# 87003697/DynamiCrafter

Measured on AMD Instinct MI355X. Metric: frames/sec (and denoising-step ms), 16f@576x1024, DDIM 50, higher is better.
Workload: dtype bf16; 1 GPU; inference_1024_v1.0.yaml: 1 clip/GPU, 16 frames, latent 72x128, DDIM 50 uniform_trailing eta=1, CFG 7.5 batched (cond+uncond), guidance_rescale 0.7, v-param+ZTSNR+dynamic rescale, hipGraph-captured step; clips_per_gpu=1, parallelism=dp1 over 1 distinct clips (no data-path collective), conditioning=local (1 rank), outputs_finite=True

## Files before the change

### dynamicrafter_amd/_hip.py

```python
import ctypes as C
import os
import threading

_HERE = os.path.dirname(os.path.abspath(__file__))
LIB_PATH = os.environ.get("DC_HIP_LIB") or os.path.join(_HERE, "csrc", "libdcrafter_hip.so")

DC_GEMM_OUT_F32 = 1
DC_GEMM_GEGLU = 2
DC_GEMM_GELU = 4


class DcGemmParams(C.Structure):
    _fields_ = [
        ("A", C.c_void_p), ("W", C.c_void_p), ("C", C.c_void_p), ("bias", C.c_void_p),
        ("rowvec", C.c_void_p), ("residual", C.c_void_p),
        ("lda", C.c_int), ("ldc", C.c_int), ("ldr", C.c_int), ("rowvec_ld", C.c_int),
        ("rows_per_vec", C.c_int),
        ("M", C.c_int), ("N", C.c_int), ("K", C.c_int), ("n_pad", C.c_int),
        ("mode", C.c_int), ("Cin", C.c_int),
        ("IH", C.c_int), ("IW", C.c_int), ("OH", C.c_int), ("OW", C.c_int),
        ("stride", C.c_int), ("pad", C.c_int), ("ups", C.c_int),
        ("T", C.c_int), ("HW", C.c_int),
        ("flags", C.c_int), ("alpha", C.c_float),
        ("workspace", C.c_void_p), ("workspace_bytes", C.c_longlong),
# ... 47 lines not shown
    _fields_ = [
        ("c1", C.c_void_p), ("c2", C.c_void_p), ("w", C.c_void_p), ("step_size", C.c_void_p), ("bc2_sqrt", C.c_void_p),
        ("step_index", C.c_void_p), ("index", C.c_int), ("weight_type", C.c_int), ("x0_param", C.c_int),
        ("e_nchw", C.c_int), ("cfg_scale", C.c_float), ("guidance_rescale", C.c_float),
        ("beta2", C.c_float), ("eps", C.c_float), ("one_minus_beta1", C.c_float), ("one_minus_beta2", C.c_float),
        ("decay", C.c_float), ("grad_scale", C.c_float), ("noise_step_stride", C.c_int64), ("loss", C.c_void_p),
    ]


_P, _I, _F, _L = C.c_void_p, C.c_int, C.c_float, C.c_int64
SIGNATURES = {
    "dc_gemm_conv": (_I, [C.POINTER(DcGemmParams), _P]),
    "dc_gemm_fit": (_I, [C.POINTER(DcGemmParams), _P]),
    "dc_gemm_fit_shape": (_I, [_I, _I, _I]),
    "dc_gemm_workspace_bytes": (_L, []),
    "dc_gemm_last_variant": (C.c_char_p, []),
    "dc_gemm_set_plan": (_I, [_I]),
    "dc_groupnorm": (_I, [_P, _I, _P, _I, _P, _P, _I, _I, _I, _I, _F, _I, _P, _P]),
    "dc_groupnorm_workspace_bytes": (_L, [_I, _I, _I]),
    "dc_layernorm": (_I, [_P, _I, _P, _I, _P, _P, _I, _I, _F, _P]),
    "dc_ln_pool_tokens": (_I, [_P, _I, _P, _I, _P, _P, _I, _I, _I, _I, _I, _I, _F, _P]),
    "dc_flash_attn_d64": (_I, [_P, _P, _P, _P, _I, _I, _I, _I, _I, _I, _I, _I, _L, _L, _F, _I, _F, _P]),
    "dc_ff_geglu_fused320": (_I, [_P, _I, _P, _P, _F, _P, _P, _P, _P, _P, _I, _P, _I, _I, _P]),
    "dc_ff_geglu_proj_fused320": (_I, [_P, _I, _P, _P, _F, _P, _P, _P, _P, _P, _P, _P, _I, _P, _I, _I, _P]),
    "dc_ln_linear": (_I, [_P, _I, _I, _P, _P, _F, _P, _P, _P, _I, _I, _I, _P]),
    "dc_ln_qkv_temporal_attn320": (_I, [_P, _I, _P, _P, _F, _P, _P, _I, _I, _I, _I, _F, _P]),
    "dc_ln_qkv_temporal_attn640": (_I, [_P, _I, _P, _P, _F, _P, _P, _I, _I, _I, _I, _F, _P]),
    "dc_gn_silu_tconv3": (_I, [_P, _I, _I, _P, _P, _P, _I, _P, _P, _P, _I, _P, _I, _I, _I, _I, _I, _P]),
    "dc_groupnorm_stats": (_I, [_P, _I, _I, _I, _I, _I, _F, _P, _P, _P]),
    "dc_gn_linear": (_I, [_P, _I, _I, _P, _P, _P, _I, _I, _P, _P, _P, _I, _I, _I, _P]),
    "dc_flash_attn_set_mode": (_I, [_I, _F]),
    "dc_linear_residual": (_I, [_P, _I, _I, _P, _P, _P, _I, _P, _I, _I, _I, _P]),
    "dc_cross_attn_dual_d64": (_I, [_P, _P, _P, _P, _P, _P, _I, _I, _I, _I, _I, _I, _I, _I, _L, _L, _F, _F, _P]),
    "dc_temporal_attn_d64": (_I, [_P, _I, _P, _I, _I, _I, _I, _I, _F, _P]),
    "dc_gemv_small": (_I, [_P, _I, _P, _P, _P, _I, _I, _I, _I, _I, _I, _I, _P]),
    "dc_timestep_embedding": (_I, [_P, _P, _I, _P, _I, _I, _F, _P]),
    "dc_pack_latent": (_I, [_P, _P, _P, _I, _I, _I, _I, _I, _I, _I, _P]),
    "dc_pack_latent_windows": (_I, [_P, _P, _P, _P, _P] + [_I] * 13 + [_P]),
    "dc_window_merge": (_I, [_P, _I, _P, _I, _P, _P, _P] + [_I] * 12 + [_P]),
    "dc_pack_latent_tiles": (_I, [_P, _P, _P, _P, _P] + [_I] * 16 + [_P]),
    "dc_tile_merge": (_I, [_P, _I, _P, _I, _P, _P, _P] + [_I] * 15 + [_P]),
    "dc_nchw_to_rows": (_I, [_P, _P, _I, _I, _I, _I, _F, _P]),
    "dc_rows_to_nchw": (_I, [_P, _I, _I, _P, _I, _I, _I, _F, _P]),
    "dc_im2col3x3_c8": (_I, [_P, _I, _P, _I, _I, _I, _I, _P]),
    "dc_copy2d": (_I, [_P, _I, _P, _I, _I, _I, _P]),
    "dc_build_context": (_I, [_P, _P, _I, _I, _I, _I, _I, _P]),
    "dc_softmax_rows": (_I, [_P, _I, _P, _I, _I, _I, _P]),
    "dc_transpose": (_I, [_P, _I, _P, _I, _I, _I, _P]),
    "dc_add_rows": (_I, [_P, _I, _P, _I, _P, _I, _I, _I, _P]),
    "dc_vae_sample": (_I, [_P, _I, _P, _P, _I, _I, _I, _F, _P]),
    "dc_ddim_step": (_I, [C.POINTER(DcDdimParams), _P, _P, _P, _I, _P, _P, _P, _P, _I, _I, _I, _P, _P]),
    "dc_ddim_invert_step": (_I, [C.POINTER(DcInvertParams), _P, _P, _P, _I, _P, _P, _P, _I, _I, _I, _P, _P]),
    "dc_dpmpp_step": (_I, [C.POINTER(DcDpmParams), _P, _P, _P, _I, _P, _P, _P, _P, _I, _I, _I, _P, _P]),
    "dc_sds_noise": (_I, [C.POINTER(DcSdsParams), _P, _P, _P, _I, _L, _P]),
    "dc_sds_step": (_I, [C.POINTER(DcSdsParams), _P, _P, _I, _P, _P, _P, _P, _I, _I, _I, _P, _P]),
    "dc_attn_small": (_I, [_P, _P, _P, _P, _I, _I, _I, _I, _I, _I, _I, _I, _I, _F, _I, _P]),
    "dc_attn_small_lds_bytes": (_L, [_I, _I]),
    "dc_clip_preprocess": (_I, [_P, _P, _P, _P, _I, _I, _I, _I, _I, _I, _I, C.POINTER(_F), C.POINTER(_F), _P]),
    "dc_patchify": (_I, [_P, _P, _I, _I, _I, _I, _I, _I, _P]),
    "dc_embed_tokens": (_I, [_P, _P, _P, _P, _I, _I, _I, _I, _P]),
    "dc_frames_to_u8": (_I, [_P, _P, _I, _I, _I, _I, _I, _P]),
    "dc_jpeg_dct_quant": (_I, [_P, _P, _P, _I, _I, _I, _P]),
    "dc_jpeg_entropy": (_I, [_P, _P, _P, _I, _I, _I, _I, _L, _P]),
    "dc_jpeg_pack": (_I, [_P, _P, _P, _P, _P, _I, _I, _L, _L, _P]),
    "dc_jpeg_decode_entropy": (_I, [_P, _L, _P, _P, _P, _P, _P] + [_I] * 8 + [_P]),
    "dc_jpeg_decode_idct": (_I, [_P, _P, _P] + [_I] * 6 + [_P]),
# ... 79 lines not shown
```

### dynamicrafter_amd/csrc/attn_parts.h

```cpp
#pragma once
#include "dc_common.h"
#include "lds_stage.h"

namespace {

constexpr int ATTN_VLD = 192;

__device__ __forceinline__ int attn_key_of(int j0, int r, int fh) { return j0 + (r & 3) + 8 * (r >> 2) + 4 * fh; }
__device__ __forceinline__ bf16x8_t attn_q_scaled(const u32x4_t& raw, float c) {
    u32x4_t sc;
#pragma unroll
    for (int e = 0; e < 4; ++e) sc[e] = pack_bf2(__uint_as_float(raw[e] << 16) * c, __uint_as_float(raw[e] & 0xffff0000u) * c);
    return __builtin_bit_cast(bf16x8_t, sc);
}
__device__ __forceinline__ bf16x8_t attn_pack_p(const f32x16_t& s, int ks) {
    u32x4_t pw;
#pragma unroll
    for (int e = 0; e < 4; ++e) pw[e] = pack_bf2(s[8 * ks + 2 * e], s[8 * ks + 2 * e + 1]);
    return __builtin_bit_cast(bf16x8_t, pw);
}
__device__ __forceinline__ int attn_vt_lane_off(int lane) {
    const int li = lane & 15;
    return (li >> 2) * ATTN_VLD + (((lane >> 4) & 1) * 16 + (li & 3) * 4) * 2;
}
__device__ __forceinline__ bf16x8_t attn_vt_join(const bf16x4_t lo, const bf16x4_t hi) {
    bf16x8_t vf;
    vf[0] = lo[0]; vf[1] = lo[1]; vf[2] = lo[2]; vf[3] = lo[3];
    vf[4] = hi[0]; vf[5] = hi[1]; vf[6] = hi[2]; vf[7] = hi[3];
    return vf;
}
__device__ __forceinline__ bf16x8_t attn_vt_frag(const lds_char_t* vp) {
    const bf16x4_t lo = __builtin_amdgcn_ds_read_tr16_b64_v4i16((lds_bf16x4_t*)(vp));
    const bf16x4_t hi = __builtin_amdgcn_ds_read_tr16_b64_v4i16((lds_bf16x4_t*)(vp + 8 * ATTN_VLD));
    return attn_vt_join(lo, hi);
}
__device__ __forceinline__ void attn_stage_row(char* sk, char* sv, int r, int chunk, const u32x4_t& kreg, const u32x4_t& vreg) {
    *reinterpret_cast<u32x4_t*>(sk + lds_off128(r, chunk)) = kreg;
    *reinterpret_cast<u32x4_t*>(sv + r * ATTN_VLD + chunk * 16) = vreg;
}
__device__ __forceinline__ void attn_store_row(bf16_t* orow, bool live, int fh, const f32x16_t (&f)[2]) {
#pragma unroll
    for (int db = 0; db < 2; ++db)
#pragma unroll
        for (int qd = 0; qd < 4; qd += 2) {
            const unsigned a0 = pack_bf2(f[db][4 * qd + 0], f[db][4 * qd + 1]);
            const unsigned a1 = pack_bf2(f[db][4 * qd + 2], f[db][4 * qd + 3]);
            const unsigned b0 = pack_bf2(f[db][4 * qd + 4], f[db][4 * qd + 5]);
            const unsigned b1 = pack_bf2(f[db][4 * qd + 6], f[db][4 * qd + 7]);
            const auto r0 = __builtin_amdgcn_permlane32_swap(a0, b0, false, false);
            const auto r1 = __builtin_amdgcn_permlane32_swap(a1, b1, false, false);
            const u32x4_t pk = {r0[0], r1[0], r0[1], r1[1]};
            if (live) *reinterpret_cast<u32x4_t*>(orow + db * 32 + 8 * (qd + fh)) = pk;
        }
}

}
```

### dynamicrafter_amd/csrc/ff_fused.hip

```cpp
#include "attn_parts.h"
#include "dc_common.h"
#include "dcrafter_hip.h"
#include "lds_stage.h"
#include <stdint.h>
#include <type_traits>

namespace {

constexpr int FD = 320;
constexpr int FM = 4 * FD;
constexpr int FCH = 32;
constexpr int FNCH = FM / FCH;
constexpr int FBM = 128;
constexpr int W1_STAGE = 64 * FD * 2;
constexpr int W2_STAGE = FD * FCH * 2;
constexpr int W2_RING = 3;
constexpr int FF_LDS = 2 * W1_STAGE + W2_RING * W2_STAGE + 4 * 2048 + 2 * FM * 4;
static_assert(FF_LDS <= 160 * 1024, "LDS");

#ifdef DC_FF_STAMPS
__device__ unsigned long long g_ff_stamps[8];
#define FF_STAMP(i) do { asm volatile("s_waitcnt lgkmcnt(0)" ::: "memory"); const unsigned long long t__ = __builtin_readcyclecounter(); \
                         st_acc[i] += t__ - st_last; st_last = t__; } while (0)
#else
// ... 936 lines not shown
                                                     : __builtin_amdgcn_update_dpp(0, __float_as_int(yv), 0x101, 0xf, 0xf, false));
                }
            }
        }
        {
            const int n0 = c * LCH;
            const int rrow = lane >> 2, rc = lane & 3;
            if constexpr (RES) {
                if constexpr (KH != 1) {
#pragma unroll
                    for (int t = 0; t < 2; ++t) rres[t] = *reinterpret_cast<const u32x4_t*>(p.R + grow(t * 16 + rrow) * p.ldr + n0 + rc * 8);
                }
#pragma unroll
                for (int t = 0; t < 2; ++t) *xs_patch_row(ebuf, t * 16 + rrow, rc) = rres[t];
            }
#pragma unroll
            for (int q = 0; q < 4; ++q) {
                float4 bv = bias_lds ? *reinterpret_cast<const float4*>(bls + n0 + 8 * q + 4 * fh)
                                     : *reinterpret_cast<const float4*>(p.bias + n0 + 8 * q + 4 * fh);
                uint2* const slot2 = xs_patch_acc(ebuf, fr, fh, q);
                if constexpr (RES) xs_add_bf16x4(bv, *slot2);
                *slot2 = xs_pack_acc(out, q, bv);
            }
#pragma unroll
            for (int t = 0; t < 2; ++t) {
                const int r = t * 16 + rrow;
                const u32x4_t d = *xs_patch_row(ebuf, r, rc);
                *reinterpret_cast<u32x4_t*>(p.O + grow(r) * p.ldo + n0 + rc * 8) = d;
            }
        }
    }
}

}

#ifdef DC_FF_STAMPS
extern "C" int dc_ff_debug_stamps(unsigned long long* out, int reset) {
    hipError_t e = hipMemcpyFromSymbol(out, HIP_SYMBOL(g_ff_stamps), sizeof(unsigned long long) * 8);
    if (e == hipSuccess && reset) {
        unsigned long long z[8] = {0};
        e = hipMemcpyToSymbol(HIP_SYMBOL(g_ff_stamps), z, sizeof(z));
    }
    return (int)e;
}
#endif

template <bool LN, bool PROJ>
static int launch_ff_fused(const FfParams& p, hipStream_t stream) {
    static DcLdsOnce lds_once;
    if (const int e = lds_once.ensure(reinterpret_cast<const void*>(&ff_geglu_fused320_kernel<LN, PROJ>), FF_LDS)) return e;
    const int tiles = (p.M + FBM - 1) / FBM;
    hipLaunchKernelGGL((ff_geglu_fused320_kernel<LN, PROJ>), dim3(tiles < 256 ? tiles : 256), dim3(256), FF_LDS, stream, p);
    DC_CHECK_LAUNCH();
    return 0;
}

static int ff_fused_common(const uint16_t* x, int ldx, const float* ln_gamma, const float* ln_beta, float ln_eps,
                           const uint16_t* w1, const float* b1, const uint16_t* w2p, const float* b2, const uint16_t* residual,
                           int ldr, uint16_t* out, int ldo, const uint16_t* wp, const float* bp, const uint16_t* residual2,
                           int ldr2, uint16_t* out2, int ldo2, int M, hipStream_t stream) {
    FfParams p;
    p.X = x; p.ldx = ldx; p.W1 = w1; p.b1 = b1; p.W2p = w2p; p.b2 = b2; p.R = residual; p.ldr = ldr; p.O = out; p.ldo = ldo;
    p.M = M; p.ln_g = ln_gamma; p.ln_b = ln_beta; p.ln_eps = ln_eps;
    p.Wp = wp; p.bp = bp; p.R2 = residual2; p.ldr2 = ldr2; p.O2 = out2; p.ldo2 = ldo2;
    if (wp) return ln_gamma ? launch_ff_fused<true, true>(p, stream) : launch_ff_fused<false, true>(p, stream);
    return ln_gamma ? launch_ff_fused<true, false>(p, stream) : launch_ff_fused<false, false>(p, stream);
// ... 50 lines not shown
    }
    if (norm == 1) return launch_norm_linear_t<1, 2>(p, grid, stream);
    if (norm == 2) return launch_norm_linear_t<2, 2>(p, grid, stream);
    return launch_norm_linear_t<0, 2>(p, grid, stream);
}

static int ll_params(LlParams& p, const uint16_t* x, int ldx, int K, const uint16_t* w, const float* bias, uint16_t* out, int ldo,
                     int M, int N) {
    if ((K != FD && K != 2 * FD) || M < 1 || N < LCH || N % LCH || ldx % 8 || ldo % 8) return DC_ERR_SHAPE;
    if (((uintptr_t)x | (uintptr_t)out | (uintptr_t)w) % 16) return DC_ERR_SHAPE;
    p.X = x; p.ldx = ldx; p.W = w; p.bias = bias; p.O = out; p.ldo = ldo; p.M = M; p.N = N;
    p.ln_g = nullptr; p.ln_b = nullptr; p.ln_eps = 0.f; p.gn_stats = nullptr; p.gn_groups = 1; p.gn_rpi = FBM;
    p.R = nullptr; p.ldr = 0;
    return 0;
}

extern "C" int dc_ln_linear(const uint16_t* x, int ldx, int K, const float* ln_gamma, const float* ln_beta, float ln_eps,
                            const uint16_t* w, const float* bias, uint16_t* out, int ldo, int M, int N, void* stream_) {
    if (!x || !w || !out || ((ln_gamma == nullptr) != (ln_beta == nullptr))) return DC_ERR_ARG;
    LlParams p;
    if (const int e = ll_params(p, x, ldx, K, w, bias, out, ldo, M, N)) return e;
    p.ln_g = ln_gamma; p.ln_b = ln_beta; p.ln_eps = ln_eps;
    return launch_norm_linear(ln_gamma ? 1 : 0, K, p, (hipStream_t)stream_);
}

extern "C" int dc_linear_residual(const uint16_t* x, int ldx, int K, const uint16_t* w, const float* bias,
                                  const uint16_t* residual, int ldr, uint16_t* out, int ldo, int M, int N, void* stream_) {
    if (!x || !w || !out || !residual) return DC_ERR_ARG;
    LlParams p;
    if (const int e = ll_params(p, x, ldx, K, w, bias, out, ldo, M, N)) return e;
    if (ldr % 8 || (uintptr_t)residual % 16) return DC_ERR_SHAPE;
    p.R = residual; p.ldr = ldr;
    return launch_norm_linear(0, K, p, (hipStream_t)stream_);
}

extern "C" int dc_gn_linear(const uint16_t* x, int ldx, int K, const float* gamma, const float* beta, const float* stats,
                            int groups, int rows_per_inst, const uint16_t* w, const float* bias, uint16_t* out, int ldo,
                            int M, int N, void* stream_) {
    if (!x || !w || !out || !gamma || !beta || !stats) return DC_ERR_ARG;
    LlParams p;
    if (const int e = ll_params(p, x, ldx, K, w, bias, out, ldo, M, N)) return e;
    if (groups < 1 || K % groups || rows_per_inst < FBM || rows_per_inst % FBM || M % rows_per_inst) return DC_ERR_SHAPE;
    p.ln_g = gamma; p.ln_b = beta;
    p.gn_stats = reinterpret_cast<const float2*>(stats); p.gn_groups = groups; p.gn_rpi = rows_per_inst;
    return launch_norm_linear(2, K, p, (hipStream_t)stream_);
}

template <int KH>
static int launch_ln_qkv_tattn(const uint16_t* x, int ldx, const float* ln_gamma, const float* ln_beta, float ln_eps,
                               const uint16_t* wqkv, uint16_t* out, int ldo, int B, int T, int HW, float scale, void* stream_) {
    if (!x || !ln_gamma || !ln_beta || !wqkv || !out) return DC_ERR_ARG;
    if (B < 1 || T != 16 || HW < 8 || HW % 8 || ldx % 8 || ldo % 8) return DC_ERR_SHAPE;
    if (((uintptr_t)x | (uintptr_t)out | (uintptr_t)wqkv) % 16) return DC_ERR_SHAPE;
    static DcLdsOnce lds_once;
    if (const int e = lds_once.ensure(reinterpret_cast<const void*>(&ln_qkv_tattn_kernel<KH>), ta_lds(KH))) return e;
    TaParams p;
    p.X = x; p.ldx = ldx; p.W = wqkv; p.O = out; p.ldo = ldo; p.ln_g = ln_gamma; p.ln_b = ln_beta; p.ln_eps = ln_eps;
    p.HW = HW; p.c = scale * 1.4426950408889634f;
    static const int hsplit_env = [] { const char* e = getenv("DC_TA_HSPLIT"); return e ? atoi(e) : 0; }();
    const int hsplit = (KH == 2 && hsplit_env == 2) ? 2 : 1;
    hipLaunchKernelGGL(ln_qkv_tattn_kernel<KH>, dim3((unsigned)(B * (HW / 8)), hsplit), dim3(256), ta_lds(KH), (hipStream_t)stream_, p);
    DC_CHECK_LAUNCH();
    return 0;
}

extern "C" int dc_ln_qkv_temporal_attn320(const uint16_t* x, int ldx, const float* ln_gamma, const float* ln_beta, float ln_eps,
// ... 40 lines not shown
```

### dynamicrafter_amd/lvdm/modules/networks/openaimodel3d.py

```python
import math

import torch
import torch.nn as nn

from .... import ops
from ....ops import PackedWeight
from ....param_tree import attach_params

import os

_BF16 = torch.bfloat16
_FF_FUSED = os.environ.get("DC_FF_FUSED", "1") != "0"
_LN_FUSED = os.environ.get("DC_LN_FUSED", "1") != "0"
_LR_FUSED = os.environ.get("DC_LR_FUSED", "1") != "0"
_TA_FUSED = os.environ.get("DC_TA_FUSED", "1") != "0"
_TA_FUSED_C = tuple(int(k) for k in os.environ.get("DC_TA_FUSED_C", "320,640").split(","))
_FFP_FUSED = os.environ.get("DC_FFP_FUSED", "1") != "0"
_TC_FUSED = os.environ.get("DC_TC_FUSED", "1") != "0"
_GEMM_FIT = os.environ.get("DC_GEMM_FIT", "1") != "0"
_FIT_ROUTES = {
    (1280, 1280): "61 / 86 [gemm_persist_kernel<128>]; with residual 79 / 95; same bits",
    (3840, 1280): "168 / 207 [gemm_persist_kernel<320>]; same bits",
}
_FIT_MEASURED_NOT_ROUTED = {
    (1280, 5120): "213 / 255 [gemm_pipe320x16_kernel+splitk]",
    (640, 2560): "251 / 316 [gemm_pipe320x16_kernel+splitk]",
    (1280, 1920): "78 / 123 [gemm_pipe320x16_kernel+splitk]",
    (1280, 2560): "100 / 143 [gemm_pipe320x16_kernel+splitk]",
}


def _linear(a, pw, out, residual=None):
    if _GEMM_FIT and (pw.N, pw.K) in _FIT_ROUTES and ops.gemm_fits(out.shape[0], pw):
        return ops.gemm_fit(a, pw, out, residual=residual)
    return ops.gemm(a, pw, out, residual=residual)
_FUSED_MIN_ROWS = int(os.environ.get("DC_FUSED_MIN_ROWS", "4096"))
_LN_FUSED_K = tuple(int(k) for k in os.environ.get("DC_LN_FUSED_K", "320,640").split(","))
C_IN_PAD = 64


def _block_layout(cfg):
    mc, mults, nrb = cfg["model_channels"], list(cfg["channel_mult"]), cfg["num_res_blocks"]
    attn_res = set(cfg["attention_resolutions"])
    hc = cfg["num_head_channels"]
    tconv = bool(cfg["temporal_conv"])

    def transformers(ch):
        out = [("spatial", {"ch": ch, "heads": ch // hc})]
        if cfg["temporal_attention"]:
            out.append(("temporal", {"ch": ch, "inner": ch, "heads": ch // hc, "linear": bool(cfg["use_linear"])}))
        return out
# ... 511 lines not shown
    def _ff_proj(self, W, h, x, out):
        B_ = W["blk"]
        if "proj_p" in W and _FF_FUSED and _FFP_FUSED and h.shape[0] >= _FUSED_MIN_ROWS:
            return ops.ff_geglu_proj_fused320(h, B_["ff1"], B_["ff2p"], B_["ff2"].bias, W["proj_p"], W["proj_out"].bias, x, out,
                                              ln=B_["norm3"], ln_eps=1e-5)
        h = self._ff(B_, h)
        return self._lin_res(h, W["proj_out"], x, out)

    def _spatial_pre(self, W, x, g, heads):
        A = self._arena
        M, dev, Cc = x.shape[0], x.device, x.shape[1]
        h = self._gn_linear(x, W["norm"], W["proj_in"], A.get("tr_h", M, Cc, device=dev), n_inst=g["F"], rpi=g["HW"])
        B_ = W["blk"]
        return self._attn_self_spatial(B_["attn1"], B_["norm1"], h, g, heads)

    def _context_kv(self, B_, ctx, tag):
        return ops.gemm(ctx, B_["kv_ctx"], self._arena.get(tag, ctx.shape[0], B_["kv_ctx"].N, device=ctx.device))

    def precompute_context_kv(self, ctx_rows):
        Wt = self.packed(ctx_rows.device)
        down_path, middle, up_path = self._layout
        out = {"__gen__": Wt["gen"]}
        for name, blks, Ws in (("in", down_path, Wt["in"]), ("mid", [middle], [Wt["mid"]]), ("out", up_path, Wt["out"])):
            for i, (blk, Wb) in enumerate(zip(blks, Ws)):
                for j, ((kind, a), W) in enumerate(zip(blk, Wb)):
                    if kind == "spatial":
                        out[W["blk"]["key"]] = self._context_kv(W["blk"], ctx_rows, f"kvctx.{name}{i}.{j}")
        return out

    def _spatial_post(self, W, x, h, g, heads, out_tag, out=None):
        A = self._arena
        M, dev, Cc = x.shape[0], x.device, x.shape[1]
        B_ = W["blk"]
        q = self._ln_linear(h, B_["norm2"], B_["q2"], A.get("q2", M, Cc, device=dev))
        kv = None if g.get("ctx_kv") is None else g["ctx_kv"].get(B_["key"])
        if kv is None:
            kv = self._context_kv(B_, g["ctx"], "kvctx")
        att = A.get("att", M, Cc, device=dev)
        Lc, nt = g["Lc"], g["n_text"]
        if self.image_cross_attention and Lc > nt:
            ops.cross_attn_dual(q, kv[:, :Cc], kv[:, Cc:2 * Cc], kv[nt:, 2 * Cc:3 * Cc], kv[nt:, 3 * Cc:], att, batch=g["F"],
                                heads=heads, Lq=g["HW"], Lk=nt, Lk2=Lc - nt, scale=0.125, scale2=B_["ip_scale"], kv_bstride=Lc)
        else:
            ops.flash_attn(q, kv[:, :Cc], kv[:, Cc:2 * Cc], att, batch=g["F"], heads=heads, Lq=g["HW"], Lk=nt, scale=0.125,
                           kv_bstride=Lc)
        h = self._lin_res(att, B_["out2"], h, h)
        return self._ff_proj(W, h, x, out if out is not None else A.get(out_tag, M, Cc, device=dev))

    def _spatial(self, W, x, g, heads, out_tag, out=None):
        return self._spatial_post(W, x, self._spatial_pre(W, x, g, heads), g, heads, out_tag, out=out)

    def _temporal(self, W, x, g, heads, out_tag, out=None):
        A = self._arena
        M, dev, Cc = x.shape[0], x.device, x.shape[1]
        inner = W["proj_in"].N
        h = self._gn_linear(x, W["norm"], W["proj_in"], A.get("tr_h", M, inner, device=dev), n_inst=g["B"],
                            rpi=g["T"] * g["HW"])
        B_ = W["blk"]
        h = self._attn_self_temporal(B_["attn1"], B_["norm1"], h, g, heads)
        h = self._attn_self_temporal(B_["attn2"], B_["norm2"], h, g, heads)
        return self._ff_proj(W, h, x, out if out is not None else A.get(out_tag, M, Cc, device=dev))

    def _run_block(self, blk, Wb, h, g, tag, final=None):
        A = self._arena
        for j, ((kind, a), W) in enumerate(zip(blk, Wb)):
            out_tag = f"{tag}.{j}"
            dev = h.device
            last = final is not None and j == len(blk) - 1
            if kind == "conv_in":
                conv = dict(IH=g["H"], IW=g["W"], OH=g["H"], OW=g["W"], stride=1, pad=1, ups=0)
                dst = final(h.shape[0], a["cout"]) if last else A.get(out_tag, h.shape[0], a["cout"], device=dev)
                if "lin8" in W:
# ... 186 lines not shown
```

### dynamicrafter_amd/ops.py

```python
import ctypes as C
import os
import math

import torch

from . import _hip
from ._hip import DcDdimParams, DcGemmParams, check

_BF16 = torch.bfloat16


def stream_ptr():
    return C.c_void_p(torch.cuda.current_stream().cuda_stream)


class Tracer:

    def __init__(self):
        self.records = []

    def __enter__(self):
        global _TRACE
        _TRACE = self
        return self
# ... 440 lines not shown
    _launch("ff_geglu_proj_fused320", 2.0 * M * (2560 + 1280 + 320) * 320, 2.0 * M * 320 * 3 + 2.0 * (2560 * 320 + 320 * 1280 + 320 * 320),
            _hip.lib().dc_ff_geglu_proj_fused320, _ptr(x), x.stride(0), _ptr(None if ln is None else ln[0]),
            _ptr(None if ln is None else ln[1]), ln_eps, _ptr(pw1.w), _ptr(pw1.bias), _ptr(w2p), _ptr(b2), _ptr(wp), _ptr(bp),
            _ptr(residual2), residual2.stride(0), _ptr(out), out.stride(0), M, stream_ptr())
    return out


def ln_linear(x, pw, out, ln=None, ln_eps=1e-5):
    _rows(x, "x"); _rows(out, "out")
    M, K = x.shape[0], pw.K
    if K not in (320, 640) or pw.N % 32:
        raise ValueError("ln_linear: K must be 320 or 640 and N a multiple of 32")
    _need_rows(x, M, K, "x"); _need_rows(out, M, pw.N, "out")
    if ln is not None:
        _need(ln[0], K, "ln gamma"); _need(ln[1], K, "ln beta")
    _launch("ln_linear", 2.0 * M * pw.N * K, 2.0 * M * (K + pw.N) + 2.0 * pw.N * K, _hip.lib().dc_ln_linear,
            _ptr(x), x.stride(0), K, _ptr(None if ln is None else ln[0]), _ptr(None if ln is None else ln[1]), ln_eps,
            _ptr(pw.w), _ptr(pw.bias), _ptr(out), out.stride(0), M, pw.N, stream_ptr())
    return out


def linear_residual(x, pw, residual, out):
    _rows(x, "x"); _rows(out, "out"); _rows(residual, "residual")
    M, K = x.shape[0], pw.K
    if K not in (320, 640) or pw.N % 32:
        raise ValueError("linear_residual: K must be 320 or 640 and N a multiple of 32")
    _need_rows(x, M, K, "x"); _need_rows(out, M, pw.N, "out"); _need_rows(residual, M, pw.N, "residual")
    _launch("linear_residual", 2.0 * M * pw.N * K, 2.0 * M * (K + 2 * pw.N) + 2.0 * pw.N * K, _hip.lib().dc_linear_residual,
            _ptr(x), x.stride(0), K, _ptr(pw.w), _ptr(pw.bias), _ptr(residual), residual.stride(0), _ptr(out), out.stride(0),
            M, pw.N, stream_ptr())
    return out


def ln_qkv_temporal_attn(x, ln, pw_qkv, out, *, B, T, HW, scale, ln_eps=1e-5):
    _rows(x, "x"); _rows(out, "out")
    M = B * T * HW
    Cc = pw_qkv.K
    if Cc not in (320, 640) or pw_qkv.N != 3 * Cc or pw_qkv.bias is not None or T != 16 or HW % 8:
        raise ValueError("ln_qkv_temporal_attn: dim 320 / 640 (qkv weight [3 C, C], no bias), T = 16, HW % 8 == 0")
    if x.data_ptr() == out.data_ptr():
        raise ValueError("ln_qkv_temporal_attn: out must not alias x")
    _need_rows(x, M, Cc, "x"); _need_rows(out, M, Cc, "out"); _need(ln[0], Cc, "ln gamma"); _need(ln[1], Cc, "ln beta")
    fn = _hip.lib().dc_ln_qkv_temporal_attn320 if Cc == 320 else _hip.lib().dc_ln_qkv_temporal_attn640
    _launch(f"ln_qkv_temporal_attn{Cc}", 2.0 * M * 3 * Cc * Cc + 4.0 * M * T * Cc, 4.0 * M * Cc + 2.0 * 3 * Cc * Cc,
            fn, _ptr(x), x.stride(0), _ptr(ln[0]), _ptr(ln[1]), ln_eps, _ptr(pw_qkv.w),
            _ptr(out), out.stride(0), B, T, HW, scale, stream_ptr())
    return out


def gn_silu_tconv3(x, gamma, beta, stats, pw, out, *, B, T, HW, groups=32, residual=None):
    _rows(x, "x"); _rows(out, "out")
    M = B * T * HW
    C = pw.w.shape[1] // 3
    if C not in (320, 640) or pw.w.shape[1] != 3 * C or pw.N % 32 or pw.bias is None or T != 16 or HW % 8:
        raise ValueError("gn_silu_tconv3: 320 / 640 input channels (weight [N, 3 C] with bias), N % 32 == 0, T = 16, HW % 8 == 0")
    if x.data_ptr() == out.data_ptr():
        raise ValueError("gn_silu_tconv3: out must not alias x")
    _need_rows(x, M, C, "x"); _need_rows(out, M, pw.N, "out")
    _need(gamma, C, "gamma"); _need(beta, C, "beta"); _need(stats, B * groups * 2, "stats")
    if residual is not None:
        _rows(residual, "residual"); _need_rows(residual, M, pw.N, "residual")
    _launch("gn_silu_tconv3", 2.0 * M * pw.N * 3 * C, 2.0 * M * (C + pw.N * (2 if residual is not None else 1)) + 2.0 * pw.N * 3 * C,
            _hip.lib().dc_gn_silu_tconv3, _ptr(x), x.stride(0), C, _ptr(gamma), _ptr(beta), _ptr(stats), groups, _ptr(pw.w),
            _ptr(pw.bias), _ptr(residual), 0 if residual is None else residual.stride(0), _ptr(out), out.stride(0), B, T, HW,
            pw.N, stream_ptr())
    return out
# ... 1099 lines not shown
```

### include/dcrafter_hip.h

```cpp
#ifndef DCRAFTER_HIP_H
#define DCRAFTER_HIP_H
#include <stdint.h>

#ifdef __cplusplus
extern "C" {
#endif

#define DC_ERR_SHAPE (-1)
#define DC_ERR_ARG   (-2)

#define DC_GEMM_OUT_F32 1
#define DC_GEMM_GEGLU   2
#define DC_GEMM_GELU    4

typedef struct DcGemmParams {
    const uint16_t* A;
    const uint16_t* W;
    void* C;
    const float* bias;
    const float* rowvec;
    const uint16_t* residual;
    int lda, ldc, ldr, rowvec_ld;
    int rows_per_vec;
    int M, N, K, n_pad;
// ... 172 lines not shown
    float grad_scale;
    int64_t noise_step_stride;
    float* loss;
} DcSdsParams;

int dc_sds_noise(const DcSdsParams* p, const float* latent, const float* noise, float* x_t, int B, int64_t n_per_clip,
                 void* stream);

int dc_sds_step(const DcSdsParams* p, const float* e_cond, const float* e_uncond, int ld_e, const float* x_t,
                float* latent, float* m, float* v, int B, int C, int THW, float* workspace, void* stream);

int dc_cross_attn_dual_d64(const uint16_t* q, const uint16_t* k, const uint16_t* v, const uint16_t* k2, const uint16_t* v2,
                           uint16_t* o, int ldq, int ldkv, int ldo, int batch, int heads, int Lq, int Lk, int Lk2,
                           int64_t q_bstride, int64_t kv_bstride, float scale, float scale2, void* stream);

int dc_ff_geglu_fused320(const uint16_t* x, int ldx, const float* ln_gamma, const float* ln_beta, float ln_eps,
                         const uint16_t* w1, const float* b1, const uint16_t* w2p, const float* b2, const uint16_t* residual,
                         int ldr, uint16_t* out, int ldo, int M, void* stream);

int dc_ff_geglu_proj_fused320(const uint16_t* x, int ldx, const float* ln_gamma, const float* ln_beta, float ln_eps,
                              const uint16_t* w1, const float* b1, const uint16_t* w2p, const float* b2, const uint16_t* wp,
                              const float* bp, const uint16_t* residual2, int ldr2, uint16_t* out, int ldo, int M, void* stream);

int dc_ln_linear(const uint16_t* x, int ldx, int K, const float* ln_gamma, const float* ln_beta, float ln_eps, const uint16_t* w,
                 const float* bias, uint16_t* out, int ldo, int M, int N, void* stream);
int dc_groupnorm_stats(const uint16_t* x, int ldx, int C, int groups, int n_inst, int rows_per_inst, float eps,
                       float* workspace, float* stats_out, void* stream);
int dc_gn_linear(const uint16_t* x, int ldx, int K, const float* gamma, const float* beta, const float* stats, int groups,
                 int rows_per_inst, const uint16_t* w, const float* bias, uint16_t* out, int ldo, int M, int N, void* stream);

int dc_linear_residual(const uint16_t* x, int ldx, int K, const uint16_t* w, const float* bias, const uint16_t* residual, int ldr,
                       uint16_t* out, int ldo, int M, int N, void* stream);

int dc_ln_qkv_temporal_attn320(const uint16_t* x, int ldx, const float* ln_gamma, const float* ln_beta, float ln_eps,
                               const uint16_t* wqkv, uint16_t* out, int ldo, int B, int T, int HW, float scale, void* stream);
int dc_ln_qkv_temporal_attn640(const uint16_t* x, int ldx, const float* ln_gamma, const float* ln_beta, float ln_eps,
                               const uint16_t* wqkv, uint16_t* out, int ldo, int B, int T, int HW, float scale, void* stream);

int dc_gn_silu_tconv3(const uint16_t* x, int ldx, int C, const float* gamma, const float* beta, const float* stats, int groups,
                      const uint16_t* w, const float* bias, const uint16_t* residual, int ldr, uint16_t* out, int ldo, int B, int T,
                      int HW, int N, void* stream);


int dc_attn_small(const uint16_t* q, const uint16_t* k, const uint16_t* v, uint16_t* o, int ldq, int ldk, int ldv, int ldo,
                  int B, int heads, int Lq, int Lk, int d, float scale, int causal, void* stream);
int64_t dc_attn_small_lds_bytes(int Lk, int d);

int dc_clip_preprocess(const float* img, float* tmp0, float* tmp1, float* out, int N, int C, int H, int W, int OH, int OW,
                       int antialias, const float* mean3, const float* std3, void* stream);

int dc_patchify(const float* img, uint16_t* rows, int N, int C, int H, int W, int p, int kpad, void* stream);

int dc_embed_tokens(const int64_t* tokens, const uint16_t* table, const uint16_t* pos, uint16_t* out, int B, int L, int D,
                    int vocab, void* stream);

int dc_frames_to_u8(const float* video, uint8_t* out, int N, int C, int T, int H, int W, void* stream);


#define DC_JPEG_MCU_MAX_BYTES 2496

int dc_jpeg_dct_quant(const uint8_t* frames, const uint8_t* qtab, int16_t* coef, int T, int H, int W, void* stream);

int dc_jpeg_entropy(const int16_t* coef, uint8_t* scratch, int32_t* seg_len, int T, int my, int mx, int ri, int64_t stride,
                    void* stream);

int dc_jpeg_pack(const uint8_t* scratch, const int32_t* seg_len, int32_t* seg_off, uint8_t* out, int32_t* frame_len, int T,
// ... 129 lines not shown
```

Baseline: 2.590 frames/s.

## Fuse LN, Q projection, dual cross-attention and output projection for C=320 blocks

Adds one kernel that handles the C=320 spatial-transformer cross-attention block. Per 128-row tile it applies LayerNorm, the to_q GEMM, text plus image dual cross-attention with K/V staged in LDS, the to_out GEMM, the bias and the residual add. This removes the q and attention-output round trips to HBM and two kernel launches per block. The cost is a large register- and LDS-heavy kernel that loops over heads serially and may lose occupancy compared with the separate kernels. It is gated by shape conditions (Lk in 65..96, image tokens at most 32, HW divisible by 128).

Result: no change. 2.608 frames/s (median of 6 runs) (+0.7%).

```diff
diff --git a/dynamicrafter_amd/_hip.py b/dynamicrafter_amd/_hip.py
--- a/dynamicrafter_amd/_hip.py
+++ b/dynamicrafter_amd/_hip.py
@@ -103,6 +103,8 @@
     "dc_flash_attn_set_mode": (_I, [_I, _F]),
     "dc_linear_residual": (_I, [_P, _I, _I, _P, _P, _P, _I, _P, _I, _I, _I, _P]),
     "dc_cross_attn_dual_d64": (_I, [_P, _P, _P, _P, _P, _P, _I, _I, _I, _I, _I, _I, _I, _I, _L, _L, _F, _F, _P]),
+    "dc_xattn_block_fused320": (_I, [_P, _I, _P, _P, _F, _P, _P, _P, _P, _P, _P, _I, _L, _I, _I, _F, _F, _P, _P, _P, _I,
+                                     _I, _I, _I, _I, _P]),
     "dc_temporal_attn_d64": (_I, [_P, _I, _P, _I, _I, _I, _I, _I, _F, _P]),
     "dc_gemv_small": (_I, [_P, _I, _P, _P, _P, _I, _I, _I, _I, _I, _I, _I, _P]),
     "dc_timestep_embedding": (_I, [_P, _P, _I, _P, _I, _I, _F, _P]),
diff --git a/dynamicrafter_amd/csrc/attn_parts.h b/dynamicrafter_amd/csrc/attn_parts.h
--- a/dynamicrafter_amd/csrc/attn_parts.h
+++ b/dynamicrafter_amd/csrc/attn_parts.h
@@ -38,6 +38,11 @@
     *reinterpret_cast<u32x4_t*>(sk + lds_off128(r, chunk)) = kreg;
     *reinterpret_cast<u32x4_t*>(sv + r * ATTN_VLD + chunk * 16) = vreg;
 }
+__device__ __forceinline__ u32x4_t attn_swap_piece(unsigned a0, unsigned a1, unsigned b0, unsigned b1) {
+    const auto r0 = __builtin_amdgcn_permlane32_swap(a0, b0, false, false);
+    const auto r1 = __builtin_amdgcn_permlane32_swap(a1, b1, false, false);
+    return u32x4_t{r0[0], r1[0], r0[1], r1[1]};
+}
 __device__ __forceinline__ void attn_store_row(bf16_t* orow, bool live, int fh, const f32x16_t (&f)[2]) {
 #pragma unroll
     for (int db = 0; db < 2; ++db)
@@ -47,9 +52,7 @@
             const unsigned a1 = pack_bf2(f[db][4 * qd + 2], f[db][4 * qd + 3]);
             const unsigned b0 = pack_bf2(f[db][4 * qd + 4], f[db][4 * qd + 5]);
             const unsigned b1 = pack_bf2(f[db][4 * qd + 6], f[db][4 * qd + 7]);
-            const auto r0 = __builtin_amdgcn_permlane32_swap(a0, b0, false, false);
-            const auto r1 = __builtin_amdgcn_permlane32_swap(a1, b1, false, false);
-            const u32x4_t pk = {r0[0], r1[0], r0[1], r1[1]};
+            const u32x4_t pk = attn_swap_piece(a0, a1, b0, b1);
             if (live) *reinterpret_cast<u32x4_t*>(orow + db * 32 + 8 * (qd + fh)) = pk;
         }
 }
diff --git a/dynamicrafter_amd/csrc/ff_fused.hip b/dynamicrafter_amd/csrc/ff_fused.hip
--- a/dynamicrafter_amd/csrc/ff_fused.hip
+++ b/dynamicrafter_amd/csrc/ff_fused.hip
@@ -992,6 +992,230 @@
     }
 }
 
+
+constexpr int XB_K1 = 0, XB_V1 = 96 * 128, XB_K2 = XB_V1 + 96 * ATTN_VLD, XB_V2 = XB_K2 + 32 * 128, XB_KV = XB_V2 + 32 * ATTN_VLD;
+static_assert(XB_KV <= 2 * LW_STAGE, "a head's K / V sets alias the weight ring");
+constexpr int XB_LDS = 2 * LW_STAGE + 4 * 2048 + 2 * FD * 4 + 2 * FD * 4;
+
+struct XbParams {
+    const bf16_t* X; int ldx;
+    const float* ln_g; const float* ln_b; float ln_eps;
+    const bf16_t* Wq; const float* bq;
+    const bf16_t* K1; const bf16_t* V1; const bf16_t* K2; const bf16_t* V2; int ldkv; int64_t kv_bstride; int Lk, Lk2;
+    float c;
+    float acc_scale;
+    const bf16_t* Wo; const float* bo;
+    bf16_t* O; int ldo;
+    int HW;
+};
+
+__global__ __launch_bounds__(256, 2)
+void xattn_block320_kernel(const XbParams p) {
+    extern __shared__ __attribute__((aligned(16))) char smem[];
+    const int tid = threadIdx.x;
+    const int lane = tid & 63;
+    const int wave = __builtin_amdgcn_readfirstlane(tid >> 6);
+    const int fr = lane & 31, fh = lane >> 5;
+    const unsigned lds_base = (unsigned)(unsigned long)((lds_char_t*)smem);
+    char* const ebuf = smem + 2 * LW_STAGE + wave * 2048;
+    float* const lns = reinterpret_cast<float*>(smem + 2 * LW_STAGE + 4 * 2048);
+    float* const bqs = lns + 2 * FD;
+    float* const bos = bqs + FD;
+    const int tile = xcd_remap(blockIdx.x, gridDim.x);
+    const int frame = (tile * FBM) / p.HW;
+    const XsRowsLinear rows{tile * FBM + wave * 32, (int)gridDim.x * FBM};
+
+    unsigned vo[5];
+    xs_piece_offsets<FD * 2, 128>(vo, wave, lane);
+    auto w_base = [&](const bf16_t* W, int c) { return (uint64_t)(uintptr_t)W + (uint64_t)c * (LCH * FD * 2); };
+    xs_issue_stage(lds_base, 0, wave, vo, w_base(p.Wq, 0));
+
+    u32x4_t qa[FD / 16];
+    constexpr int PD = 6;
+    {
+        bf16x8_t xf[FD / 16];
+        xs_load_rows(xf, p.X + rows(fr) * p.ldx + fh * 8);
+        xs_stage_ln_affine(lns, FD, p.ln_g, p.ln_b, tid);
+        if (p.bq) xs_stage_bias(bqs, p.bq, FD, tid);
+        if (p.bo) xs_stage_bias(bos, p.bo, FD, tid);
+        asm volatile("s_waitcnt vmcnt(0) lgkmcnt(0)" ::: "memory");
+        __builtin_amdgcn_s_barrier();
+        asm volatile("" ::: "memory");
+        ln_rows_inplace<FD>(xf, lns, lns + FD, p.ln_eps, fh);
+#pragma unroll
+        for (int c = 0; c < FD / LCH; ++c) {
+            if (c > 0) {
+                wait_vmcnt<0>();
+                __builtin_amdgcn_s_barrier();
+                asm volatile("" ::: "memory");
+            }
+            f32x16_t acc;
+#pragma unroll
+            for (int r = 0; r < 16; ++r) acc[r] = 0.f;
+            const bool more = c + 1 < FD / LCH;
+            const uint64_t nb = w_base(p.Wq, c + 1);
+            xs_stage_mma<PD>(smem + (c & 1) * LW_STAGE, xf, 0, acc, fr, fh, [&](int i) __attribute__((always_inline)) {
+                if (more) lds_dma16_sbase(xs_stage_dst(lds_base, ((c & 1) ^ 1) * LW_STAGE, wave, i), vo[i], nb);
+            });
+#pragma unroll
+            for (int qd = 0; qd < 4; qd += 2) {
+                float4 bv0 = {0.f, 0.f, 0.f, 0.f}, bv1 = {0.f, 0.f, 0.f, 0.f};
+                if (p.bq) {
+                    bv0 = *reinterpret_cast<const float4*>(bqs + c * LCH + 8 * qd + 4 * fh);
+                    bv1 = *reinterpret_cast<const float4*>(bqs + c * LCH + 8 * (qd + 1) + 4 * fh);
+                }
+                const uint2 a = xs_pack_acc(acc, qd, bv0), b = xs_pack_acc(acc, qd + 1, bv1);
+                qa[2 * c + (qd >> 1)] = attn_swap_piece(a.x, a.y, b.x, b.y);
+            }
+        }
+    }
+
+    const int tr_off = attn_vt_lane_off(lane);
+    auto scores = [&](const char* sk, int nkeys, auto NB_, f32x16_t (&s)[3], const bf16x8_t (&qf)[4]) __attribute__((always_inline)) -> float {
+        constexpr int NB = decltype(NB_)::value;
+#pragma unroll
+        for (int jb = 0; jb < NB; ++jb) {
+#pragma unroll
+            for (int r = 0; r < 16; ++r) s[jb][r] = 0.f;
+#pragma unroll
+            for (int kk = 0; kk < 4; ++kk) {
+                const bf16x8_t kf = *reinterpret_cast<const bf16x8_t*>(sk + lds_off128(jb * 32 + fr, kk * 2 + fh));
+                s[jb] = __builtin_amdgcn_mfma_f32_32x32x16_bf16(kf, qf[kk], s[jb], 0, 0, 0);
+            }
+        }
+#pragma unroll
+        for (int r = 0; r < 16; ++r)
+            if (attn_key_of((NB - 1) * 32, r, fh) >= nkeys) s[NB - 1][r] = -1e30f;
+        float mx = s[0][0];
+#pragma unroll
+        for (int jb = 0; jb < NB; ++jb)
+#pragma unroll
+            for (int r = 0; r < 16; ++r) mx = fmaxf(mx, s[jb][r]);
+        mx = fmaxf(mx, __shfl_xor(mx, 32, 64));
+        float sum = 0.f;
+#pragma unroll
+        for (int jb = 0; jb < NB; ++jb)
+#pragma unroll
+            for (int r = 0; r < 16; ++r) {
+                const float pv = __builtin_amdgcn_exp2f(s[jb][r] - mx);
+                s[jb][r] = pv;
+                sum += pv;
+            }
+        return sum + __shfl_xor(sum, 32, 64);
+    };
+    auto pv_mma = [&](const char* sv, auto NB_, const f32x16_t (&s)[3], f32x16_t (&oacc)[2]) __attribute__((always_inline)) {
+        constexpr int NB = decltype(NB_)::value;
+#pragma unroll
+        for (int jb = 0; jb < NB; ++jb)
+#pragma unroll
+            for (int ks = 0; ks < 2; ++ks) {
+                const int jbase = jb * 32 + 16 * ks + 4 * fh;
+                const bf16x8_t pf = attn_pack_p(s[jb], ks);
+#pragma unroll
+                for (int db = 0; db < 2; ++db) {
+                    const bf16x8_t vf = attn_vt_frag((const lds_char_t*)(sv + jbase * ATTN_VLD + db * 64 + tr_off));
+                    oacc[db] = __builtin_amdgcn_mfma_f32_32x32x16_bf16(vf, pf, oacc[db], 0, 0, 0);
+                }
+            }
+    };
+    {
+        const int chunk = tid & 7, srow = tid >> 3;
+        const size_t kvrow0 = (size_t)frame * p.kv_bstride;
+#pragma unroll
+        for (int head = 0; head < FD / 64; ++head) {
+            u32x4_t kr[4], vr[4];
+#pragma unroll
+            for (int i = 0; i < 3; ++i) {
+                int j = srow + 32 * i;
+                j = j < p.Lk ? j : p.Lk - 1;
+                kr[i] = *reinterpret_cast<const u32x4_t*>(p.K1 + (kvrow0 + j) * p.ldkv + head * 64 + chunk * 8);
+                vr[i] = *reinterpret_cast<const u32x4_t*>(p.V1 + (kvrow0 + j) * p.ldkv + head * 64 + chunk * 8);
+            }
+            {
+                const int j = srow < p.Lk2 ? srow : p.Lk2 - 1;
+                kr[3] = *reinterpret_cast<const u32x4_t*>(p.K2 + (kvrow0 + j) * p.ldkv + head * 64 + chunk * 8);
+                vr[3] = *reinterpret_cast<const u32x4_t*>(p.V2 + (kvrow0 + j) * p.ldkv + head * 64 + chunk * 8);
+            }
+            __builtin_amdgcn_s_barrier();
+            asm volatile("" ::: "memory");
+#pragma unroll
+            for (int i = 0; i < 3; ++i) attn_stage_row(smem + XB_K1, smem + XB_V1, srow + 32 * i, chunk, kr[i], vr[i]);
+            attn_stage_row(smem + XB_K2, smem + XB_V2, srow, chunk, kr[3], vr[3]);
+            __syncthreads();
+
+            bf16x8_t qf[4];
+#pragma unroll
+            for (int kk = 0; kk < 4; ++kk) qf[kk] = attn_q_scaled(qa[4 * head + kk], p.c);
+            f32x16_t s[3], o1[2], o2[2];
+#pragma unroll
+            for (int d = 0; d < 2; ++d)
+#pragma unroll
+                for (int r = 0; r < 16; ++r) { o1[d][r] = 0.f; o2[d][r] = 0.f; }
+            const float l1 = scores(smem + XB_K1, p.Lk, ic<3>{}, s, qf);
+            pv_mma(smem + XB_V1, ic<3>{}, s, o1);
+            const float l2 = scores(smem + XB_K2, p.Lk2, ic<1>{}, s, qf);
+            pv_mma(smem + XB_V2, ic<1>{}, s, o2);
+            const float w1 = 1.0f / l1, w2 = p.acc_scale / l2;
+#pragma unroll
+            for (int db = 0; db < 2; ++db)
+#pragma unroll
+                for (int qd = 0; qd < 4; qd += 2) {
+                    float f[8];
+#pragma unroll
+                    for (int e = 0; e < 8; ++e) f[e] = __builtin_fmaf(o1[db][4 * qd + e], w1, o2[db][4 * qd + e] * w2);
+                    const unsigned a0 = pack_bf2(f[0], f[1]), a1 = pack_bf2(f[2], f[3]);
+                    const unsigned b0 = pack_bf2(f[4], f[5]), b1 = pack_bf2(f[6], f[7]);
+                    qa[4 * head + 2 * db + (qd >> 1)] = attn_swap_piece(a0, a1, b0, b1);
+                }
+        }
+    }
+
+    {
+        bf16x8_t xf[FD / 16];
+#pragma unroll
+        for (int kk = 0; kk < FD / 16; ++kk) xf[kk] = __builtin_bit_cast(bf16x8_t, qa[kk]);
+        __builtin_amdgcn_s_barrier();
+        asm volatile("" ::: "memory");
+        xs_issue_stage(lds_base, 0, wave, vo, w_base(p.Wo, 0));
+        int slot = 0;
+        for (int c = 0; c < FD / LCH; ++c) {
+            if (c == 0) wait_vmcnt<0>();
+            else wait_vmcnt<2>();
+            __builtin_amdgcn_s_barrier();
+            asm volatile("" ::: "memory");
+            f32x16_t acc;
+#pragma unroll
+            for (int r = 0; r < 16; ++r) acc[r] = 0.f;
+            u32x4_t rres[2];
+            xs_load_chunk_rows(rres, p.X, p.ldx, rows, c * LCH, lane);
+            const bool more = c + 1 < FD / LCH;
+            const uint64_t nb = w_base(p.Wo, c + 1);
+            xs_stage_mma<PD>(smem + slot * LW_STAGE, xf, 0, acc, fr, fh, [&](int i) __attribute__((always_inline)) {
+                if (more) lds_dma16_sbase(xs_stage_dst(lds_base, (slot ^ 1) * LW_STAGE, wave, i), vo[i], nb);
+            });
+            slot ^= 1;
+            const int n0 = c * LCH;
+            const int rrow = lane >> 2, rc = lane & 3;
+#pragma unroll
+            for (int t = 0; t < 2; ++t) *xs_patch_row(ebuf, t * 16 + rrow, rc) = rres[t];
+#pragma unroll
+            for (int q = 0; q < 4; ++q) {
+                float4 bv = {0.f, 0.f, 0.f, 0.f};
+                if (p.bo) bv = *reinterpret_cast<const float4*>(bos + n0 + 8 * q + 4 * fh);
+                uint2* const pslot = xs_patch_acc(ebuf, fr, fh, q);
+                xs_add_bf16x4(bv, *pslot);
+                *pslot = xs_pack_acc(acc, q, bv);
+            }
+#pragma unroll
+            for (int t = 0; t < 2; ++t) {
+                const int r = t * 16 + rrow;
+                const u32x4_t d = *xs_patch_row(ebuf, r, rc);
+                *reinterpret_cast<u32x4_t*>(p.O + rows(r) * p.ldo + n0 + rc * 8) = d;
+            }
+        }
+    }
+}
+
 }
 
 #ifdef DC_FF_STAMPS
@@ -1108,6 +1332,30 @@
     if (ldr % 8 || (uintptr_t)residual % 16) return DC_ERR_SHAPE;
     p.R = residual; p.ldr = ldr;
     return launch_norm_linear(0, K, p, (hipStream_t)stream_);
+}
+
+extern "C" int dc_xattn_block_fused320(const uint16_t* h, int ldh, const float* ln_gamma, const float* ln_beta, float ln_eps,
+                                       const uint16_t* wq, const float* bq, const uint16_t* k, const uint16_t* v,
+                                       const uint16_t* k2, const uint16_t* v2, int ldkv, int64_t kv_bstride, int Lk, int Lk2,
+                                       float scale, float scale2, const uint16_t* wo, const float* bo, uint16_t* out, int ldo,
+                                       int C, int heads, int F, int HW, void* stream_) {
+    if (!h || !ln_gamma || !ln_beta || !wq || !k || !v || !k2 || !v2 || !wo || !out) return DC_ERR_ARG;
+    if (C != FD || heads != FD / 64 || F < 1 || HW < FBM || HW % FBM) return DC_ERR_SHAPE;
+    if (Lk <= 64 || Lk > 96 || Lk2 < 1 || Lk2 > 32 || kv_bstride < 0) return DC_ERR_SHAPE;
+    if (ldh % 8 || ldo % 8 || ldkv % 8 || ldh < FD || ldo < FD) return DC_ERR_SHAPE;
+    if (((uintptr_t)h | (uintptr_t)out | (uintptr_t)wq | (uintptr_t)wo | (uintptr_t)k | (uintptr_t)v | (uintptr_t)k2 | (uintptr_t)v2) % 16)
+        return DC_ERR_SHAPE;
+    const long long tiles = (long long)F * (HW / FBM);
+    if (tiles * FBM > 0x7fffffffLL) return DC_ERR_SHAPE;
+    static DcLdsOnce lds_once;
+    if (const int e = lds_once.ensure(reinterpret_cast<const void*>(&xattn_block320_kernel), XB_LDS)) return e;
+    XbParams p;
+    p.X = h; p.ldx = ldh; p.ln_g = ln_gamma; p.ln_b = ln_beta; p.ln_eps = ln_eps; p.Wq = wq; p.bq = bq;
+    p.K1 = k; p.V1 = v; p.K2 = k2; p.V2 = v2; p.ldkv = ldkv; p.kv_bstride = kv_bstride; p.Lk = Lk; p.Lk2 = Lk2;
+    p.c = scale * 1.4426950408889634f; p.acc_scale = scale2; p.Wo = wo; p.bo = bo; p.O = out; p.ldo = ldo; p.HW = HW;
+    hipLaunchKernelGGL(xattn_block320_kernel, dim3((unsigned)tiles), dim3(256), XB_LDS, (hipStream_t)stream_, p);
+    DC_CHECK_LAUNCH();
+    return 0;
 }
 
 extern "C" int dc_gn_linear(const uint16_t* x, int ldx, int K, const float* gamma, const float* beta, const float* stats,
diff --git a/dynamicrafter_amd/lvdm/modules/networks/openaimodel3d.py b/dynamicrafter_amd/lvdm/modules/networks/openaimodel3d.py
--- a/dynamicrafter_amd/lvdm/modules/networks/openaimodel3d.py
+++ b/dynamicrafter_amd/lvdm/modules/networks/openaimodel3d.py
@@ -17,6 +17,7 @@
 _TA_FUSED_C = tuple(int(k) for k in os.environ.get("DC_TA_FUSED_C", "320,640").split(","))
 _FFP_FUSED = os.environ.get("DC_FFP_FUSED", "1") != "0"
 _TC_FUSED = os.environ.get("DC_TC_FUSED", "1") != "0"
+_XA_BLOCK_FUSED = os.environ.get("DC_XATTN_BLOCK_FUSED", "1") != "0"
 _GEMM_FIT = os.environ.get("DC_GEMM_FIT", "1") != "0"
 _FIT_ROUTES = {
     (1280, 1280): "61 / 86 [gemm_persist_kernel<128>]; with residual 79 / 95; same bits",
@@ -594,12 +595,20 @@
         A = self._arena
         M, dev, Cc = x.shape[0], x.device, x.shape[1]
         B_ = W["blk"]
-        q = self._ln_linear(h, B_["norm2"], B_["q2"], A.get("q2", M, Cc, device=dev))
+        Lc, nt = g["Lc"], g["n_text"]
+        fused = (_XA_BLOCK_FUSED and Cc == 320 and self.image_cross_attention and Lc > nt and 64 < nt <= 96 and Lc - nt <= 32
+                 and M >= _FUSED_MIN_ROWS and g["HW"] % 128 == 0 and g["HW"] >= 512)
+        if not fused:
+            q = self._ln_linear(h, B_["norm2"], B_["q2"], A.get("q2", M, Cc, device=dev))
         kv = None if g.get("ctx_kv") is None else g["ctx_kv"].get(B_["key"])
         if kv is None:
             kv = self._context_kv(B_, g["ctx"], "kvctx")
+        if fused:
+            h = ops.xattn_block_fused320(h, B_["norm2"], B_["q2"], kv[:, :Cc], kv[:, Cc:2 * Cc], kv[nt:, 2 * Cc:3 * Cc],
+                                         kv[nt:, 3 * Cc:], B_["out2"], h, F=g["F"], HW=g["HW"], heads=heads, Lk=nt, Lk2=Lc - nt,
+                                         scale=0.125, scale2=B_["ip_scale"], kv_bstride=Lc)
+            return self._ff_proj(W, h, x, out if out is not None else A.get(out_tag, M, Cc, device=dev))
         att = A.get("att", M, Cc, device=dev)
-        Lc, nt = g["Lc"], g["n_text"]
         if self.image_cross_attention and Lc > nt:
             ops.cross_attn_dual(q, kv[:, :Cc], kv[:, Cc:2 * Cc], kv[nt:, 2 * Cc:3 * Cc], kv[nt:, 3 * Cc:], att, batch=g["F"],
                                 heads=heads, Lq=g["HW"], Lk=nt, Lk2=Lc - nt, scale=0.125, scale2=B_["ip_scale"], kv_bstride=Lc)
diff --git a/dynamicrafter_amd/ops.py b/dynamicrafter_amd/ops.py
--- a/dynamicrafter_amd/ops.py
+++ b/dynamicrafter_amd/ops.py
@@ -496,6 +496,26 @@
     return out
 
 
+def xattn_block_fused320(h, ln, pw_q, k, v, k2, v2, pw_o, out, *, F, HW, heads, Lk, Lk2, scale, scale2, kv_bstride, ln_eps=1e-5):
+    for t, n in ((h, "h"), (out, "out"), (k, "k"), (v, "v"), (k2, "k2"), (v2, "v2")):
+        _rows(t, n)
+    if len({k.stride(0), v.stride(0), k2.stride(0), v2.stride(0)}) != 1:
+        raise ValueError("xattn_block_fused320: k, v, k2, v2 must share one row stride")
+    M, Cc = F * HW, pw_q.K
+    if pw_q.N != Cc or pw_o.N != Cc or pw_o.K != Cc:
+        raise ValueError("xattn_block_fused320: to_q and to_out must be square and of one width")
+    _need_rows(h, M, Cc, "h"); _need_rows(out, M, Cc, "out")
+    _need(ln[0], Cc, "ln gamma"); _need(ln[1], Cc, "ln beta")
+    _need_rows(k, (F - 1) * kv_bstride + Lk, heads * 64, "k"); _need_rows(v, (F - 1) * kv_bstride + Lk, heads * 64, "v")
+    _need_rows(k2, (F - 1) * kv_bstride + Lk2, heads * 64, "k2"); _need_rows(v2, (F - 1) * kv_bstride + Lk2, heads * 64, "v2")
+    _launch("xattn_block_fused320", 4.0 * M * Cc * Cc + 4.0 * M * (Lk + Lk2) * heads * 64,
+            2.0 * M * Cc * 2 + 2.0 * 2 * Cc * Cc + 2.0 * F * heads * 64 * 2 * (Lk + Lk2), _hip.lib().dc_xattn_block_fused320,
+            _ptr(h), h.stride(0), _ptr(ln[0]), _ptr(ln[1]), ln_eps, _ptr(pw_q.w), _ptr(pw_q.bias), _ptr(k), _ptr(v), _ptr(k2),
+            _ptr(v2), k.stride(0), kv_bstride, Lk, Lk2, scale, scale2, _ptr(pw_o.w), _ptr(pw_o.bias), _ptr(out), out.stride(0),
+            Cc, heads, F, HW, stream_ptr())
+    return out
+
+
 def ln_qkv_temporal_attn(x, ln, pw_qkv, out, *, B, T, HW, scale, ln_eps=1e-5):
     _rows(x, "x"); _rows(out, "out")
     M = B * T * HW
diff --git a/include/dcrafter_hip.h b/include/dcrafter_hip.h
--- a/include/dcrafter_hip.h
+++ b/include/dcrafter_hip.h
@@ -228,6 +228,12 @@
 int dc_linear_residual(const uint16_t* x, int ldx, int K, const uint16_t* w, const float* bias, const uint16_t* residual, int ldr,
                        uint16_t* out, int ldo, int M, int N, void* stream);
 
+int dc_xattn_block_fused320(const uint16_t* h, int ldh, const float* ln_gamma, const float* ln_beta, float ln_eps,
+                            const uint16_t* wq, const float* bq, const uint16_t* k, const uint16_t* v, const uint16_t* k2,
+                            const uint16_t* v2, int ldkv, int64_t kv_bstride, int Lk, int Lk2, float scale, float scale2,
+                            const uint16_t* wo, const float* bo, uint16_t* out, int ldo, int C, int heads, int F, int HW,
+                            void* stream);
+
 int dc_ln_qkv_temporal_attn320(const uint16_t* x, int ldx, const float* ln_gamma, const float* ln_beta, float ln_eps,
                                const uint16_t* wqkv, uint16_t* out, int ldo, int B, int T, int HW, float scale, void* stream);
 int dc_ln_qkv_temporal_attn640(const uint16_t* x, int ldx, const float* ln_gamma, const float* ln_beta, float ln_eps,
```
